# omerkurt-okt/buck-gnn

Hardware: AMD Instinct MI355X
Metric: graphs/sec (fwd+bwd) 6-layer SAGE h=512, ~5k-node meshes, batch 16, 1/2/4/8 GPU (higher is better)
Workload: dtype f32

## Files before the change

### buck-gnn_amd/bgnn/_lib.py

```python
from __future__ import annotations

import ctypes
import os
import threading

_HERE = os.path.dirname(os.path.abspath(__file__))
LIB_PATH = os.environ.get("BGNN_LIBRARY") or os.path.join(_HERE, "_lib", "libbgnn.so")
ABI_VERSION = 16

_lock = threading.Lock()
_lib = None

c_p = ctypes.c_void_p
c_i32 = ctypes.c_int32
c_i64 = ctypes.c_int64
c_f32 = ctypes.c_float
c_u64 = ctypes.c_uint64
c_sz = ctypes.c_size_t


class CsrStruct(ctypes.Structure):

    _fields_ = [
        ("rowptr", c_p),
        ("col", c_p),
        ("heavy_row", c_p),
        ("heavy_chunk0", c_p),
        ("chunk_heavy", c_p),
        ("n_rows", c_i64),
        ("nnz", c_i64),
        ("n_heavy", c_i32),
# ... 100 lines not shown
                                     c_p]),
    "bgnn_gemm_ws_bytes_ex": (c_sz, [c_i64, c_i64, c_i64, c_i32, c_i32, c_i32]),
    "bgnn_gemm_gather_add": (c_i32, [c_i32, c_i32, c_i64, c_i64, c_i64, c_p, c_i64, c_p, c_i64, c_p, c_i64, c_p, c_i32,
                                     c_p, c_p, c_i64, c_p, c_p, c_i64, c_i32, c_p, c_sz, c_p]),
    "bgnn_absmax_f32": (c_i32, [c_p, c_i64, c_i64, c_i64, c_p, c_i32, c_p]),
    "bgnn_gemm_f32_ex": (c_i32, [c_i32, c_i32, c_i64, c_i64, c_i64, c_f32, c_p, c_i64, c_p, c_i64, c_f32, c_p,
                                 c_i64, c_p, c_i32, c_p, c_sz, c_p]),
    "bgnn_topk_rank": (c_i32, [c_p, c_p, c_p, c_i64, c_p, c_p]),
    "bgnn_topk_select": (c_i32, [c_p, c_p, c_p, c_p, c_i64, c_p, c_p, c_p, c_p]),
    "bgnn_gather_scale": (c_i32, [c_p, c_i64, c_i32, c_p, c_p, c_i64, c_p, c_i64, c_p]),
    "bgnn_gather_scale_bwd": (c_i32, [c_p, c_i64, c_p, c_i64, c_i32, c_p, c_p, c_i64, c_p, c_i64, c_p, c_p]),
    "bgnn_filter_edges_ws_bytes": (c_sz, [c_i64]),
    "bgnn_filter_edges": (c_i32, [c_p, c_i64, c_p, c_i64, c_p, c_p, c_p, c_p, c_sz, c_p]),
    "bgnn_mlp2_supported": (c_i32, [c_i32, c_i32, c_i32]),
    "bgnn_mlp2_fwd": (c_i32, [c_p, c_i64, c_i32, c_i32, c_i32, c_p, c_p, c_p, c_p, c_p, c_p, c_p]),
    "bgnn_mlp2_bwd_ws_bytes": (c_sz, [c_i64]),
    "bgnn_mlp2_bwd": (c_i32, [c_p, c_i64, c_i32, c_i32, c_i32, c_p, c_p, c_p, c_p, c_p, c_p, c_p, c_p, c_p, c_p,
                              c_sz, c_p]),
    "bgnn_gemm_f32_dropadd": (c_i32, [c_i32, c_i32, c_i64, c_i64, c_i64, c_p, c_i64, c_p, c_i64, c_p, c_i64, c_p,
                                      c_p, c_p, c_i64, c_f32, c_u64, c_p, c_sz, c_p]),
    "bgnn_gemm_f32_dropadd_cols": (c_i32, [c_i64, c_i64, c_i64, c_p, c_i64, c_p, c_i64, c_p, c_i64, c_p, c_p, c_p,
                                           c_i64, c_i64, c_f32, c_u64, c_p, c_sz, c_p]),
    "bgnn_add_dropout": (c_i32, [c_p, c_p, c_i64, c_f32, c_u64, c_p, c_p]),
    "bgnn_gemm_f32": (c_i32, [c_i32, c_i32, c_i64, c_i64, c_i64, c_f32, c_p, c_i64, c_p, c_i64, c_f32, c_p, c_i64,
                              c_p, c_sz, c_p]),
}


class BgnnError(RuntimeError):
    def __init__(self, fn: str, code: int, msg: str):
        super().__init__(f"{fn} failed with code {code}: {msg}")
        self.code = code


def load():
    global _lib
    if _lib is not None:
        return _lib
    with _lock:
        if _lib is not None:
            return _lib
        if not os.path.exists(LIB_PATH):
            raise ImportError(
                f"bgnn: native library not found at {LIB_PATH}; build it with "
                "`python -c 'import __graft_entry__ as g; g.build()'` or `make -C buck-gnn_amd`")
        lib = ctypes.CDLL(LIB_PATH)
# ... 32 lines not shown
```

### buck-gnn_amd/bgnn/fused.py

```python
from __future__ import annotations

import torch

from . import _lib
from .graph import Graph, _stream, require_cuda

GEMM_BACKEND = "hip"

PLANE_TILE = 128
Z_PLANES = False
DZ_PLANES = False
DGRAD_WT = True
FOLD_WEIGHTS_TORCH = False
DGRAD_DROPADD = True

BF16_PREP = True
ABSMAX_ITEMS = True
PERSISTENT_WPACK = True
MAX_MERGED = True
WSPLIT = True

TIMERS = None
TIMER_EVENT = None


class _timed:
    __slots__ = ("name", "ev")

    def __init__(self, name):
        self.name = name
        self.ev = None

    def __enter__(self):
        if TIMERS is not None:
            mk = TIMER_EVENT or (lambda: torch.cuda.Event(enable_timing=True))
            self.ev = (mk(), mk())
# ... 507 lines not shown
              float(cfg.p), cfg.seed, N, H, x_next.data_ptr(), next_amax.data_ptr(), None, None, s)
    return x_next, (scale, shift, mean, invstd)


def _glue_bwd_stats(g, o, scale, shift, mean, invstd, cfg: LayerConfig, g_rows=None):
    if not cfg.bn:
        return None, None, None, None
    N, H = o.shape
    dev = o.device
    s = _stream()
    rs = _lib.query("bgnn_rows_slots", N)
    part2 = torch.empty(rs, 2, H, dtype=torch.float32, device=dev)
    _lib.call("bgnn_sage_bwd_stats", g.data_ptr(), _ptr(g_rows), o.data_ptr(), scale.data_ptr(), shift.data_ptr(),
              mean.data_ptr(), invstd.data_ptr(), float(cfg.p), cfg.seed, N, H, part2.data_ptr(), s)
    sums = torch.empty(2, H, dtype=torch.float32, device=dev)
    _lib.call("bgnn_reduce_partials", part2.data_ptr(), rs, H, sums[0].data_ptr(), sums[1].data_ptr(), 0, s)
    dbeta, dgamma = sums[0], sums[1]
    if cfg.training:
        return dgamma, dbeta, sums[0], sums[1]
    z = torch.zeros(H, dtype=torch.float32, device=dev)
    return dgamma, dbeta, z, z


class SageLayerFn(torch.autograd.Function):

    @staticmethod
    def forward(ctx, x_prev, x_amax, w_l, b_l, w_r, gamma, beta, running_mean, running_var, graph: Graph,
                cfg: LayerConfig, amax=None, w_in=None, b_in=None, wprep=None, pool=None):
        dev = x_prev.device
        x_prev = x_prev.contiguous()
        H = w_l.size(0)
        N = x_prev.size(0)
        if isinstance(wprep, WPrep):
            wcat, wcat_t_pre, img_f, img_d = wprep.wcat, wprep.wcat_t, wprep, wprep
        elif wprep is not None:
            (wcat, wcat_t_pre), img_f, img_d = wprep, None, None
        else:
            wcat, wcat_t_pre, img_f, img_d = torch.cat([w_l, w_r], 0).contiguous(), None, None, None
        img_f = img_f if (img_f is not None and img_f.img_f is not None) else None
        img_d = img_d if (img_d is not None and img_d.img_d is not None) else None
        if amax is None:
            amax = torch.zeros(3, dtype=torch.float32, device=dev)
        w_amax, next_amax, dz_amax = amax[0:1], amax[1:2], amax[2:3]
        folded = w_in is not None
        if folded:
            if cfg.skip:
                raise ValueError("sage_layer: a folded input transform needs a layer without skip")
            if FOLD_WEIGHTS_TORCH:
                wf = torch.mm(wcat, w_in)
                bf = torch.mv(wcat, b_in)
            else:
                fs = cfg.famax
                fa = (fs[0:1], fs[1:2], fs[2:3]) if fs is not None else (None, None, None)
                if fs is not None:
                    absmax(wcat, fa[0], accumulate=True)
                    absmax(w_in, fa[1], accumulate=True)
                    absmax(b_in.view(1, -1), fa[2], accumulate=True)
                wf = gemm(wcat, w_in.contiguous(), trans_a=False, trans_b=False, a_amax=fa[0], b_amax=fa[1])
                bf = gemm(wcat, b_in.contiguous().view(H, 1), trans_a=False, trans_b=False, a_amax=fa[0],
                          b_amax=fa[2]).view(-1)
            absmax(wf, w_amax, accumulate=True)
            wmat = wf
        else:
            if wprep is None:
                absmax(wcat, w_amax, accumulate=True)
            wmat, bf = wcat, None
        if x_amax is None:
            x_amax = absmax(x_prev)
        planes = Z_PLANES and H % PLANE_TILE == 0 and not folded
        rng = cfg.rng
        x_full = rng.x_full if (rng is not None and rng.x_full is not None and not folded and not planes) else None
        if x_full is not None and x_full.data_ptr() != x_prev.data_ptr():
            raise RuntimeError("sage_layer: RangeRows.x_full must start at x_prev")
        xa, a_amax_g = (x_full, rng.x_amax) if x_full is not None else (x_prev, x_amax)
        M = xa.size(0)
        with _timed("gemm_fwd_fold" if folded else "gemm_fwd"):
            if planes:
                z = torch.empty(2, N, H, dtype=torch.float32, device=dev)
                gemm(x_prev, wmat, trans_a=False, trans_b=True, out=Planes(z), a_amax=x_amax, b_amax=w_amax)
                zl, zr, ldz = z[0], z[1], H
            elif (img_f is not None and not folded
                  and _lib.query("bgnn_gemm_w_tile", M, 2 * H, H) == img_f.bn_f):
                z = torch.empty(M, 2 * H, dtype=torch.float32, device=dev)
                _lib.call("bgnn_gemm_f32_w", M, 2 * H, H, xa.data_ptr(), xa.stride(0), img_f.img_f.data_ptr(),
# ... 4 lines not shown
                z = gemm(xa, wmat, trans_a=False, trans_b=True, bias=bf, a_amax=a_amax_g, b_amax=w_amax)
                zl, zr, ldz = z, z[:, H:], 2 * H
        hagg = z[N:] if x_full is not None else None
        o = torch.empty(N, H, dtype=torch.float32, device=dev)
        nrm = torch.empty(N, dtype=torch.float32, device=dev)
        slots = _lib.query("bgnn_sage_fwd_slots", graph.fwd.ref())
        bn_part = torch.empty(slots, 2, H, dtype=torch.float32, device=dev)
        part = (torch.empty(graph.fwd.plan.n_chunks * H, dtype=torch.float32, device=dev)
                if graph.fwd.plan.n_chunks else None)
        s = _stream()
        with _timed("sage_fwd"):
            _lib.call("bgnn_sage_fwd", graph.fwd.ref(), zl.data_ptr(), ldz, zr.data_ptr(), ldz, b_l.data_ptr(), H,
                      cfg.reduce, o.data_ptr(), nrm.data_ptr(), bn_part.data_ptr(), _ptr(part), _ptr(hagg),
                      2 * H if hagg is not None else 0, s)
        del z, zl, zr, hagg
        x_next, (scale, shift, mean, invstd) = _glue_fwd(o, bn_part, slots, x_prev, gamma, beta, running_mean,
                                                         running_var, cfg, next_amax, graph)
        ctx.graph = graph
        ctx.cfg = cfg
        ctx.folded = folded
        ctx.wcat_t = wcat_t_pre
        ctx.img_d = img_d if not folded else None
        ctx.set_materialize_grads(False)
        ctx.fold = (w_in, b_in, wf) if folded else None
        ctx.save_for_backward(x_prev, o, nrm, wcat, gamma if gamma is not None else torch.empty(0, device=dev),
                              scale if scale is not None else torch.empty(0, device=dev),
                              shift if shift is not None else torch.empty(0, device=dev),
                              mean if mean is not None else torch.empty(0, device=dev),
                              invstd if invstd is not None else torch.empty(0, device=dev),
                              x_amax, w_amax, dz_amax)
        ctx.mark_non_differentiable(next_amax)
        ctx.pool = pool
        if pool is not None:
            from .ops import spmm_fwd
            pooled, _ = spmm_fwd(pool.fwd, x_next, 1, pool.num_rows)
            return x_next, next_amax, pooled
        return x_next, next_amax

    @staticmethod
    def backward(ctx, g, _g_amax, g_pool=None):
        cfg: LayerConfig = ctx.cfg
        g_rows = None
        if g_pool is not None:
            seg = ctx.pool
            gp = g_pool.contiguous() / seg.fwd.degree().clamp_min(1).to(g_pool.dtype).unsqueeze(1)
            if g is None and not cfg.skip:
                g, g_rows = gp, seg.index
# ... 28 lines not shown
              if rb else None)
        _lib.call("bgnn_sage_bwd_rows", g.data_ptr(), _ptr(g_rows), o.data_ptr(), nrm.data_ptr(),
                  _ptr(scale) if bn else None, _ptr(shift) if bn else None,
                  _ptr(gamma) if (bn and gamma.numel()) else None,
                  _ptr(mean) if bn else None, _ptr(invstd) if bn else None, _ptr(sum_g2), _ptr(sum_g2xhat),
                  float(cfg.p), cfg.seed, int(cfg.skip and not dropadd), N, H, dh.data_ptr(), lddz, _ptr(gskip),
                  part_db.data_ptr(), dz_amax.data_ptr(), graph.fwd.rowptr.data_ptr() if ctx.folded else None,
                  (2 if cfg.reduce == 1 else 1) if ctx.folded else 0, _ptr(bw.ranges) if rb else None,
                  graph.fwd.rowptr.data_ptr() if (rb and cfg.reduce == 1) else None, _ptr(rp), s)
        if rb:
            _lib.call("bgnn_range_sums_finish", rp.data_ptr(), N, H, bw.ref(), 1, dzl.data_ptr(), lddz, None,
                      dz_amax.data_ptr(), s)
        db2 = torch.empty(2 if ctx.folded else 1, H, dtype=torch.float32, device=dev)
        _lib.call("bgnn_reduce_partials", part_db.data_ptr(), rs, H, db2[-1].data_ptr(),
                  db2[0].data_ptr() if ctx.folded else None, 0, s)
        db, db_zl = db2[-1], (db2[0] if ctx.folded else None)
        part = torch.empty(bw.plan.n_chunks * H, dtype=torch.float32, device=dev) if bw.plan.n_chunks else None
        with _timed("spmm_bwd"):
            _lib.call("bgnn_spmm_bwd", bw.ref(), graph.perm_t.data_ptr(), graph.fwd.rowptr.data_ptr(),
                      dh.data_ptr(), lddz, H, cfg.reduce, dzl.data_ptr(), lddz, _ptr(part),
                      dz_amax.data_ptr(), int(rb), s)
        has_affine = bn and gamma.numel() > 0
        if ctx.folded:
            w_in, b_in, wf = ctx.fold
            wf_t = wf.t().contiguous() if DGRAD_WT else wf
            with _timed("gemm_dgrad_fold"):
                dx = gemm(dz, wf_t, trans_a=False, trans_b=DGRAD_WT, a_amax=dz_amax, b_amax=w_amax)
            fs = cfg.famax
            fa = (fs[0:1], fs[1:2], fs[2:3], fs[3:4], fs[4:5]) if fs is not None else (None,) * 5
            with _timed("gemm_wgrad_fold"):
                dwf = gemm(dz, x_prev, trans_a=True, trans_b=False, a_amax=dz_amax, b_amax=x_amax,
                           c_amax=fa[3])
            dbf = db2.view(-1)
            if fs is not None:
                absmax(db2, fa[4], accumulate=True)
            if FOLD_WEIGHTS_TORCH:
                dw = torch.addmm(torch.outer(dbf, b_in), dwf, w_in.t())
                dw_in = torch.mm(wcat.t(), dwf)
                db_in = torch.mv(wcat.t(), dbf)
            else:
                dw = gemm(dwf, w_in.contiguous(), trans_a=False, trans_b=True, a_amax=fa[3],
                          b_amax=fa[1])
                dw.add_(torch.outer(dbf, b_in))
                dw_in = gemm(wcat, dwf, trans_a=True, trans_b=False, a_amax=fa[0], b_amax=fa[3])
                db_in = gemm(wcat, dbf.view(-1, 1), trans_a=True, trans_b=False, a_amax=fa[0],
                             b_amax=fa[4]).view(-1)
            return (dx, None, dw[:H], db, dw[H:], dgamma if has_affine else None, dbeta if has_affine else None,
                    None, None, None, None, None, dw_in, db_in, None, None)
        wcat_t = (ctx.wcat_t if ctx.wcat_t is not None else wcat.t().contiguous()) if DGRAD_WT else wcat
        img_d = ctx.img_d if (not planes and DGRAD_WT) else None
        if (img_d is not None and (dropadd or gskip is None)
                and _lib.query("bgnn_gemm_w_tile", N, H, 2 * H) == img_d.bn_d):
            dx = torch.empty(N, H, dtype=torch.float32, device=dev)
            with _timed("gemm_dgrad"):
                _lib.call("bgnn_gemm_f32_w", N, H, 2 * H, dz.data_ptr(), lddz, img_d.img_d.data_ptr(), img_d.bn_d,
                          dx.data_ptr(), H, None, 0, dz_amax.data_ptr(), w_amax.data_ptr(), None,
                          g.data_ptr() if dropadd else None, H, float(cfg.p) if dropadd else 0.0,
                          cfg.seed if dropadd else 0, s)
        elif dropadd:
# ... 503 lines not shown
```

### buck-gnn_amd/csrc/gemm.hip

```cpp
#include "common.h"
#include "gemm_common.h"

namespace bgnn {

extern int g_x6_bdma;

template <int KCONTIG, int BK>
struct Pad {
    static constexpr int value = KCONTIG ? (BK == 16 ? 2 : 1) : 4;
};

template <int KCONTIG, int R, int BK, int NT, bool FULL = false>
__device__ __forceinline__ void load_slice(const float* __restrict__ P, int64_t ld, int64_t Rlim, int64_t r0,
                                           int64_t k0, int64_t kend, bool vec_ok, float (&reg)[R * BK / 4 / NT][4]) {
    constexpr int NL = R * BK / 4 / NT;
    const int t = threadIdx.x;
#pragma unroll
    for (int i = 0; i < NL; ++i) {
        const int idx = t + NT * i;
        if constexpr (FULL) {
            const int r = KCONTIG ? idx / (BK / 4) : (idx % (R / 4)) * 4;
            const int k = KCONTIG ? (idx % (BK / 4)) * 4 : idx / (R / 4);
            const float* src = KCONTIG ? P + (r0 + r) * ld + (k0 + k) : P + (k0 + k) * ld + (r0 + r);
            const float4 v = *reinterpret_cast<const float4*>(src);
// ... 331 lines not shown
        p.prec = 1;
        p.cfg = g_gemm_cfg >= 0 ? g_gemm_cfg % kNumX6Cfgs : pick_x6_cfg(M, N, K, p.prec, ta == 0 && tb == 1);
        if (p.cfg == 5 && !(ta == 0 && tb == 1)) p.cfg = 1;
#ifdef BGNN_H3P_ABLATION
        if (wb && g_x6_bdma == 4 && g_gemm_cfg < 0 && N % 128 == 0 && K % 32 == 0) p.cfg = 0;
#endif
        if (!planes_ok(kX6Cfgs[p.cfg].bm, kX6Cfgs[p.cfg].bn, 32)) {
            p.cfg = 0;
            for (int c = 1; c <= 2; ++c)
                if (planes_ok(kX6Cfgs[c].bm, kX6Cfgs[c].bn, 32)) { p.cfg = c; break; }
        }
        p.bm = kX6Cfgs[p.cfg].bm; p.bn = kX6Cfgs[p.cfg].bn; p.bk = 32;
        p.split = choose_split(M, N, K, GemmCfg{p.bm, p.bn, p.bk, kX6Cfgs[p.cfg].waves,
                                                 kX6Cfgs[p.cfg].blocks_per_cu});
        return p;
    } else {
        p.cfg = pick_cfg(M, N, K, ta, tb);
        if (!planes_ok(kCfgs[p.cfg].bm, kCfgs[p.cfg].bn, kCfgs[p.cfg].bk)) p.cfg = 0;
        const GemmCfg& c = kCfgs[p.cfg];
        p.bm = c.bm; p.bn = c.bn; p.bk = c.bk;
        p.split = choose_split(M, N, K, c);
    }
    return p;
}

constexpr size_t kAmaxHead = 256;

static size_t ws_need(const Plan& p, int64_t M, int64_t N) {
    const size_t head = (p.x6 && p.prec == 1) ? kAmaxHead : 0;
    return head + (p.split > 1 ? (size_t)p.split * (size_t)M * (size_t)N * sizeof(float) : 0);
}

static int launch_splitk_reduce(float* slabs, int split, int64_t M, int64_t N, float alpha, float beta, float* C,
                                int64_t ldc, const float* bias, int relu, int64_t c_blk, int64_t c_pstride,
                                hipStream_t s) {
    int64_t blocks = (M * N + 255) / 256;
    if (blocks > 4096) blocks = 4096;
    int stride = 1;
    const int64_t eb = (M * N + 255) / 256;
    if (split >= 16 && eb < 512) {
        int64_t groups = (512 + eb - 1) / eb;
        if (groups > split / 4) groups = split / 4;
        if (groups >= 2) {
            stride = (int)((split + groups - 1) / groups);
            groups = (split + stride - 1) / stride;
            hipLaunchKernelGGL(k_splitk_stage1, dim3((unsigned)eb, (unsigned)groups), dim3(256), 0, s, slabs, split,
// ... 193 lines not shown
        GemmArgs gb{A, B, C, nullptr, M, N, K, lda, ldb, ldc, 1.f, 0.f, K, 1, bias, relu,
                    0, 0, 0, 0, nullptr, nullptr, nullptr};
        gb.st = st;
        if (b16_ok(gb, ta, tb)) {
            launch_b16(s, gb);
            BGNN_CHECK_LAUNCH();
            return BGNN_OK;
        }
    }
    const int64_t Ma = M;
    GemmArgs g{A, B, C, slabs, Ma, N, K, lda, ldb, ldc, alpha, beta, 0, split, bias, relu,
               a_blk, a_pstride, c_blk, c_pstride, a_amax, b_amax, nullptr};
    g.st = st;
    if (bs.src) {
        g.bsrc = bs.src;
        g.ld_bsrc = bs.ld;
        g.dseed = bs.seed;
        g.dthr = dropout_threshold(bs.p);
        g.dkeep = g.dthr ? 1.f / (1.f - bs.p) : 1.f;
        g.bsrc_c0 = bs.c0;
    }
    const bool c_amax_fused = c_amax != nullptr && pl.x6 && split == 1;
    if (c_amax_fused) g.c_amax = c_amax;
    int64_t kc = (K + split - 1) / split;
    kc = (kc + pl.bk - 1) / pl.bk * pl.bk;
    g.kchunk = kc > 0 ? kc : pl.bk;
    const int64_t tiles_a = ((Ma + pl.bm - 1) / pl.bm) * ((N + pl.bn - 1) / pl.bn);
    dim3 grid((unsigned)tiles_a, split);
    if (pl.x6) launch_x6(pl.prec, ta, tb, pl.cfg, bs.src ? 8 : 0, grid, s, g);
    else if (ta == 0 && tb == 0) launch_cfg<0, 0>(pl.cfg, grid, s, g);
    else if (ta == 0 && tb == 1) launch_cfg<0, 1>(pl.cfg, grid, s, g);
    else if (ta == 1 && tb == 0) launch_cfg<1, 0>(pl.cfg, grid, s, g);
    else launch_cfg<1, 1>(pl.cfg, grid, s, g);
    BGNN_CHECK_LAUNCH();
    if (split > 1) {
        const int rc = launch_splitk_reduce(slabs, split, M, N, alpha, beta, C, ldc, bias, relu, c_blk, c_pstride, s);
        if (rc != BGNN_OK) return rc;
    }
    if (c_amax != nullptr && !c_amax_fused) {
        launch_absmax(C, M, N, ldc, c_blk, c_pstride, c_amax, s);
        BGNN_CHECK_LAUNCH();
    }
    return BGNN_OK;
}

extern "C" int bgnn_gemm_f32_planes(int32_t ta, int32_t tb, int64_t M, int64_t N, int64_t K, float alpha,
                                    const float* A, int64_t lda, int64_t a_blk, int64_t a_pstride, const float* B,
                                    int64_t ldb, float beta, float* C, int64_t ldc, int64_t c_blk,
                                    int64_t c_pstride, const float* bias, int32_t relu, void* ws, size_t ws_bytes,
// ... 140 lines not shown
```

### buck-gnn_amd/csrc/gemm_common.h

```cpp
#pragma once
#include "common.h"

namespace bgnn {

typedef float floatx16 __attribute__((ext_vector_type(16)));
typedef float floatx4 __attribute__((ext_vector_type(4)));

struct GemmArgs {
    const float* A;
    const float* B;
    float* C;
    float* ws;
    int64_t M, N, K, lda, ldb, ldc;
    float alpha, beta;
    int64_t kchunk;
    int split;
    const float* bias;
    int relu;
    int64_t a_blk, a_pstride, c_blk, c_pstride;
    const float* a_amax;
    const float* b_amax;
    float* c_amax;
    const float* ga0; const int64_t* gi0; int64_t ldg0;
    const float* ga1; const int64_t* gi1; int64_t ldg1;
// ... 17 lines not shown
__device__ __forceinline__ void beta_mask4(const GemmArgs& g, int64_t row, int64_t col, const float4& t,
                                           float (&pv)[4]) {
    const int64_t i = row * g.ld_bsrc + col - g.bsrc_c0;
    const uint32_t m = g.dthr ? keep_bits4(g.dseed, (uint64_t)(i >> 2), g.dthr) : 0xFu;
    const float kf = g.dthr ? g.dkeep : 1.f;
    pv[0] = (m & 1u) ? t.x * kf : 0.f;
    pv[1] = (m & 2u) ? t.y * kf : 0.f;
    pv[2] = (m & 4u) ? t.z * kf : 0.f;
    pv[3] = (m & 8u) ? t.w * kf : 0.f;
}

__device__ __forceinline__ const float* plane_base(const float* P, int64_t x0, int64_t blk, int64_t pstride) {
    if (blk <= 0) return P;
    const int64_t plane = x0 / blk;
    return P + plane * (pstride - blk);
}

struct X6Cfg {
    int bm, bn, waves, blocks_per_cu;
};
extern const X6Cfg kX6Cfgs[];
extern const int kNumX6Cfgs;
void launch_x6(int prec, int ta, int tb, int cfg, int abl, dim3 grid, hipStream_t s, const GemmArgs& g);
bool b16_ok(const GemmArgs& g, int ta, int tb);
void launch_b16(hipStream_t s, const GemmArgs& g);
bool b16_dropadd_ok(const GemmArgs& g);
void launch_absmax(const float* P, int64_t rows, int64_t cols, int64_t ld, int64_t blk, int64_t pstride,
                   float* out, hipStream_t s);

}
```

### include/bgnn.h

```cpp
#ifndef BGNN_H
#define BGNN_H

#include <stddef.h>
#include <stdint.h>

#ifdef __cplusplus
extern "C" {
#endif

#define BGNN_ABI_VERSION 16

#define BGNN_OK 0
#define BGNN_E_ARG 1001
#define BGNN_E_WS 1002
#define BGNN_E_UNSUPPORTED 1003

#define BGNN_REDUCE_SUM 0
#define BGNN_REDUCE_MEAN 1
#define BGNN_REDUCE_MAX 2

int bgnn_abi_version(void);
const char* bgnn_last_error_string(void);

#define BGNN_TUNE_SEG_KERNEL 1
#define BGNN_TUNE_SEG_BLOCKS 2
#define BGNN_TUNE_SEG_U 3
#define BGNN_TUNE_SEG_NT 4
#define BGNN_TUNE_GEMM_MODE 5
#define BGNN_TUNE_ROWS_NT 6
#define BGNN_TUNE_GROUP_BLOCKS 7
#define BGNN_TUNE_ROWS_REV 13
#define BGNN_TUNE_GEMM_BDMA 16
int bgnn_heavy_timing(int32_t enable);
// ... 176 lines not shown
                               int64_t ldb, float* C, int64_t ldc, const float* a_amax, const float* b_amax,
                               const float* src, int64_t ld_src, int64_t src_col0, float p, uint64_t seed, void* ws,
                               size_t ws_bytes, void* stream);
int32_t bgnn_gemm_w_tile(int64_t M, int64_t N, int64_t K);
size_t bgnn_gemm_wsplit_bytes(int64_t N, int64_t K);
int bgnn_gemm_wsplit(const float* W, int32_t n_items, int64_t item_stride, int64_t N, int64_t K, int64_t ldw,
                     const float* amax, int64_t amax_stride, void* img, int64_t img_stride, int32_t bn,
                     void* stream);
int bgnn_gemm_f32_w(int64_t M, int64_t N, int64_t K, const float* A, int64_t lda, const void* wimg, int32_t bn,
                    float* C, int64_t ldc, const float* bias, int32_t relu, const float* a_amax,
                    const float* b_amax, float* c_amax, const float* src, int64_t ld_src, float p, uint64_t seed,
                    void* stream);
size_t bgnn_gemm_ws_bytes_ex(int64_t M, int64_t N, int64_t K, int32_t trans_a, int32_t trans_b,
                             int32_t precision);
int bgnn_gemm_gather_add(int32_t trans_a, int32_t trans_b, int64_t M, int64_t N, int64_t K,
                         const float* A, int64_t lda, const float* B, int64_t ldb, float* C, int64_t ldc,
                         const float* bias, int32_t relu, const float* add0, const int64_t* idx0, int64_t ld0,
                         const float* add1, const int64_t* idx1, int64_t ld1, int32_t precision,
                         void* ws, size_t ws_bytes, void* stream);
int bgnn_absmax_f32(const float* x, int64_t rows, int64_t cols, int64_t ld, float* out,
                    int32_t accumulate, void* stream);
int bgnn_absmax_items_f32(const float* x, int32_t n_items, int64_t item_stride, int64_t rows, int64_t cols,
                          int64_t ld, float* out, int64_t out_stride, void* stream);
int bgnn_gemm_f32_planes(int32_t trans_a, int32_t trans_b, int64_t M, int64_t N, int64_t K,
                         float alpha, const float* A, int64_t lda, int64_t a_blk, int64_t a_pstride,
                         const float* B, int64_t ldb, float beta, float* C, int64_t ldc,
                         int64_t c_blk, int64_t c_pstride, const float* bias, int32_t relu,
                         void* ws, size_t ws_bytes, void* stream);

int bgnn_store_gather_graph(const int64_t* table, int32_t B, int64_t Nb, int64_t Eb,
                            int64_t max_nodes, int64_t max_edges,
                            const int32_t* edge_index, int64_t ld_ei,
                            const int32_t* rowptr, const int32_t* col,
                            const int32_t* rowptr_t, const int32_t* col_t, const int32_t* perm_t,
                            int64_t* edge_index_out, int32_t* rowptr_out, int32_t* col_out,
                            int32_t* rowptr_t_out, int32_t* col_t_out, int32_t* perm_t_out,
                            int64_t* batch_out, void* stream);
int bgnn_store_gather_groups(const int64_t* gtable, int32_t B, int32_t group_rows, int64_t Nb, int64_t Gb,
                             int64_t max_edges, int64_t max_groups,
                             const int32_t* gsrc, const uint8_t* gmask, const int32_t* gcnt,
                             const int32_t* gsrc_t, const uint8_t* gmask_t, const int32_t* gcnt_t,
                             int32_t* gsrc_out, uint8_t* gmask_out, int32_t* gcnt_out,
                             int32_t* gsrc_t_out, uint8_t* gmask_t_out, int32_t* gcnt_t_out,
                             int32_t* grow_out, void* stream);
int bgnn_store_gather_rows(const int64_t* table, int32_t B, int32_t per_edge, int64_t max_rows,
                           const void* src, int64_t row_bytes, void* dst, void* stream);
// ... 52 lines not shown
```

Baseline: 2080.

## Fuse folded-input weight products into grouped native HIP kernels

Adds a native fold-weights path that computes the folded weight and bias products, their absmax, and the transposed copy in a single grouped multi-problem kernel launch, with a separate launch for operand maxima. The backward pass does the same for dW, dW_in and db_in, using split-K slabs and a reduce kernel. This replaces several separate gemm, absmax and transpose launches per folded layer. The cost removed is launch count and redundant passes over small weight matrices. It adds a large amount of new kernel code and extra workspace allocations.

```diff
diff --git a/buck-gnn_amd/bgnn/_lib.py b/buck-gnn_amd/bgnn/_lib.py
--- a/buck-gnn_amd/bgnn/_lib.py
+++ b/buck-gnn_amd/bgnn/_lib.py
@@ -6,7 +6,7 @@
 
 _HERE = os.path.dirname(os.path.abspath(__file__))
 LIB_PATH = os.environ.get("BGNN_LIBRARY") or os.path.join(_HERE, "_lib", "libbgnn.so")
-ABI_VERSION = 16
+ABI_VERSION = 17
 
 _lock = threading.Lock()
 _lib = None
@@ -153,6 +153,12 @@
     "bgnn_gemm_f32_dropadd_cols": (c_i32, [c_i64, c_i64, c_i64, c_p, c_i64, c_p, c_i64, c_p, c_i64, c_p, c_p, c_p,
                                            c_i64, c_i64, c_f32, c_u64, c_p, c_sz, c_p]),
     "bgnn_add_dropout": (c_i32, [c_p, c_p, c_i64, c_f32, c_u64, c_p, c_p]),
+    "bgnn_fold_weights_supported": (c_i32, [c_i64, c_i64]),
+    "bgnn_fold_weights_ws_bytes": (c_sz, [c_i64, c_i64]),
+    "bgnn_fold_weights_fwd": (c_i32, [c_i64, c_i64, c_p, c_i64, c_p, c_i64, c_p, c_p, c_p, c_i64, c_p, c_p, c_i64,
+                                      c_p, c_p]),
+    "bgnn_fold_weights_bwd": (c_i32, [c_i64, c_i64, c_p, c_i64, c_p, c_p, c_i64, c_p, c_i64, c_p, c_p, c_p, c_i64,
+                                      c_p, c_i64, c_p, c_p, c_sz, c_p]),
     "bgnn_gemm_f32": (c_i32, [c_i32, c_i32, c_i64, c_i64, c_i64, c_f32, c_p, c_i64, c_p, c_i64, c_f32, c_p, c_i64,
                               c_p, c_sz, c_p]),
 }
diff --git a/buck-gnn_amd/bgnn/fused.py b/buck-gnn_amd/bgnn/fused.py
--- a/buck-gnn_amd/bgnn/fused.py
+++ b/buck-gnn_amd/bgnn/fused.py
@@ -12,6 +12,7 @@
 DZ_PLANES = False
 DGRAD_WT = True
 FOLD_WEIGHTS_TORCH = False
+FOLD_NATIVE = True
 DGRAD_DROPADD = True
 
 BF16_PREP = True
@@ -565,6 +566,12 @@
     return dgamma, dbeta, z, z
 
 
+def _fold_native_ok(famax, wcat, w_in, b_in) -> bool:
+    return bool(FOLD_NATIVE and GEMM_BACKEND == "hip" and famax is not None and famax.is_contiguous()
+                and famax.numel() >= 5 and wcat.stride(1) == 1 and w_in.stride(1) == 1 and b_in.is_contiguous()
+                and _lib.query("bgnn_fold_weights_supported", wcat.size(1), w_in.size(1)))
+
+
 class SageLayerFn(torch.autograd.Function):
 
     @staticmethod
@@ -589,9 +596,19 @@
         if folded:
             if cfg.skip:
                 raise ValueError("sage_layer: a folded input transform needs a layer without skip")
+            wf_t = None
+            fold_native = not FOLD_WEIGHTS_TORCH and _fold_native_ok(cfg.famax, wcat, w_in, b_in)
             if FOLD_WEIGHTS_TORCH:
                 wf = torch.mm(wcat, w_in)
                 bf = torch.mv(wcat, b_in)
+            elif fold_native:
+                K_in = w_in.size(1)
+                wf = torch.empty(2 * H, K_in, dtype=torch.float32, device=dev)
+                bf = torch.empty(2 * H, dtype=torch.float32, device=dev)
+                wf_t = torch.empty(K_in, 2 * H, dtype=torch.float32, device=dev) if DGRAD_WT else None
+                _lib.call("bgnn_fold_weights_fwd", H, K_in, wcat.data_ptr(), wcat.stride(0), w_in.data_ptr(),
+                          w_in.stride(0), b_in.data_ptr(), cfg.famax.data_ptr(), wf.data_ptr(), K_in, bf.data_ptr(),
+                          _ptr(wf_t), 2 * H, w_amax.data_ptr(), _stream())
             else:
                 fs = cfg.famax
                 fa = (fs[0:1], fs[1:2], fs[2:3]) if fs is not None else (None, None, None)
@@ -602,7 +619,8 @@
                 wf = gemm(wcat, w_in.contiguous(), trans_a=False, trans_b=False, a_amax=fa[0], b_amax=fa[1])
                 bf = gemm(wcat, b_in.contiguous().view(H, 1), trans_a=False, trans_b=False, a_amax=fa[0],
                           b_amax=fa[2]).view(-1)
-            absmax(wf, w_amax, accumulate=True)
+            if not fold_native:
+                absmax(wf, w_amax, accumulate=True)
             wmat = wf
         else:
             if wprep is None:
@@ -653,7 +671,7 @@
         ctx.wcat_t = wcat_t_pre
         ctx.img_d = img_d if not folded else None
         ctx.set_materialize_grads(False)
-        ctx.fold = (w_in, b_in, wf) if folded else None
+        ctx.fold = (w_in, b_in, wf, wf_t) if folded else None
         ctx.save_for_backward(x_prev, o, nrm, wcat, gamma if gamma is not None else torch.empty(0, device=dev),
                               scale if scale is not None else torch.empty(0, device=dev),
                               shift if shift is not None else torch.empty(0, device=dev),
@@ -728,8 +746,8 @@
                       dz_amax.data_ptr(), int(rb), s)
         has_affine = bn and gamma.numel() > 0
         if ctx.folded:
-            w_in, b_in, wf = ctx.fold
-            wf_t = wf.t().contiguous() if DGRAD_WT else wf
+            w_in, b_in, wf, wf_t = ctx.fold
+            wf_t = (wf_t if wf_t is not None else wf.t().contiguous()) if DGRAD_WT else wf
             with _timed("gemm_dgrad_fold"):
                 dx = gemm(dz, wf_t, trans_a=False, trans_b=DGRAD_WT, a_amax=dz_amax, b_amax=w_amax)
             fs = cfg.famax
@@ -738,9 +756,21 @@
                 dwf = gemm(dz, x_prev, trans_a=True, trans_b=False, a_amax=dz_amax, b_amax=x_amax,
                            c_amax=fa[3])
             dbf = db2.view(-1)
-            if fs is not None:
+            fold_native = not FOLD_WEIGHTS_TORCH and _fold_native_ok(fs, wcat, w_in, b_in) and dwf.stride(1) == 1
+            if fs is not None and not fold_native:
                 absmax(db2, fa[4], accumulate=True)
-            if FOLD_WEIGHTS_TORCH:
+            if fold_native:
+                K_in = w_in.size(1)
+                dw = torch.empty(2 * H, H, dtype=torch.float32, device=dev)
+                dw_in = torch.empty(H, K_in, dtype=torch.float32, device=dev)
+                db_in = torch.empty(H, dtype=torch.float32, device=dev)
+                ws_bytes = _lib.query("bgnn_fold_weights_ws_bytes", H, K_in)
+                ws = torch.empty(ws_bytes, dtype=torch.uint8, device=dev) if ws_bytes else None
+                _lib.call("bgnn_fold_weights_bwd", H, K_in, dwf.data_ptr(), dwf.stride(0), dbf.data_ptr(),
+                          wcat.data_ptr(), wcat.stride(0), w_in.data_ptr(), w_in.stride(0), b_in.data_ptr(),
+                          fs.data_ptr(), dw.data_ptr(), H, dw_in.data_ptr(), K_in, db_in.data_ptr(), _ptr(ws),
+                          ws_bytes, s)
+            elif FOLD_WEIGHTS_TORCH:
                 dw = torch.addmm(torch.outer(dbf, b_in), dwf, w_in.t())
                 dw_in = torch.mm(wcat.t(), dwf)
                 db_in = torch.mv(wcat.t(), dbf)
diff --git a/buck-gnn_amd/csrc/fold.hip b/buck-gnn_amd/csrc/fold.hip
--- /dev/null
+++ b/buck-gnn_amd/csrc/fold.hip
@@ -0,0 +1,417 @@
+#include "gemm_x6_kernel.h"
+
+namespace bgnn {
+
+constexpr int FNT = 256;
+constexpr int FSL = 4;
+constexpr int f_u4(int rows) { return 2 * rows * 4; }
+
+struct FoldProb {
+    const float* A;
+    const float* B;
+    float* C;
+    float* slabs;
+    int64_t M, N, K, lda, ldb, ldc, kchunk;
+    int split, ta, tb;
+    const float* a_amax;
+    const float* b_amax;
+    int tiles_n, tiles, wg0;
+};
+
+struct FoldArgs {
+    FoldProb p[3];
+    int np;
+    float alpha;
+    float* c_amax;
+    float* ct;
+    int64_t ldct;
+    const float* ou;
+    const float* ov;
+    const float* vmax_src;
+    int64_t vmax_n;
+};
+
+__device__ __forceinline__ bool dev_aligned16(const void* p) { return ((uintptr_t)p & 15) == 0; }
+
+template <int KC, int R>
+struct FoldStage {
+    static constexpr int NQ = R * FSL / FNT;
+    static_assert(KC || (NQ >= 1 && R * FSL % FNT == 0), "k-major operand: whole quads per thread");
+    float v[KC ? FSL : NQ][KC ? x6_nu(R, FNT) : 4][8];
+
+    __device__ __forceinline__ void load(const float* __restrict__ P, int64_t ld, int64_t Rlim, int64_t r0, int64_t k0,
+                                         int64_t s0, int64_t nk, int64_t ke, bool vec_ok, int t) {
+        if constexpr (KC) {
+#pragma unroll
+            for (int u = 0; u < FSL; ++u)
+                if (s0 + u < nk) x6_load<1, R, FNT, false>(P, ld, Rlim, r0, k0 + (s0 + u) * X6_BK, ke, vec_ok, v[u], t);
+        } else {
+#pragma unroll
+            for (int j = 0; j < NQ; ++j) {
+                const int g = t + FNT * j, u = g / R, q = g % R;
+                if (s0 + u < nk) kq_load<R, false>(P, ld, Rlim, r0, k0 + (s0 + u) * X6_BK, ke, vec_ok, v[j], q);
+            }
+        }
+    }
+    __device__ __forceinline__ void store(uint4* __restrict__ S, int stride, int64_t s0, int64_t nk, float sc, int t) {
+        if constexpr (KC) {
+#pragma unroll
+            for (int u = 0; u < FSL; ++u)
+                if (s0 + u < nk) x6_store<1, R, FNT, 1>(S + u * stride, v[u], t, sc);
+        } else {
+#pragma unroll
+            for (int j = 0; j < NQ; ++j) {
+                const int g = t + FNT * j, u = g / R, q = g % R;
+                if (s0 + u < nk) kq_store<R, 1>(S + u * stride, v[j], q, sc);
+            }
+        }
+    }
+};
+
+template <int WM, int WN, int AK, int BK>
+__device__ __forceinline__ void fold_mainloop(const FoldProb& P, int64_t m0, int64_t n0, int64_t kb, int64_t ke,
+                                              float sa, float sb, uint4* __restrict__ smem, bool active,
+                                              floatx16 (&acc)[1][1]) {
+    constexpr int BM = 32 * WM, BN = 32 * WN, A_U4 = f_u4(BM), B_U4 = f_u4(BN);
+    const int t = threadIdx.x, lane = t & 63, wave = t >> 6, wm = wave / WN, wn = wave % WN;
+    const int li = lane & 31, lh = lane >> 5;
+    const bool a_vec = dev_aligned16(P.A) && P.lda % 4 == 0;
+    const bool b_vec = dev_aligned16(P.B) && P.ldb % 4 == 0;
+    const int64_t nk = ke > kb ? (ke - kb + X6_BK - 1) / X6_BK : 0;
+    FoldStage<AK, BM> ra;
+    FoldStage<BK, BN> rb;
+    ra.load(P.A, P.lda, P.M, m0, kb, 0, nk, ke, a_vec, t);
+    rb.load(P.B, P.ldb, P.N, n0, kb, 0, nk, ke, b_vec, t);
+    for (int64_t s0 = 0; s0 < nk; s0 += FSL) {
+        ra.store(smem, A_U4 + B_U4, s0, nk, sa, t);
+        rb.store(smem + A_U4, A_U4 + B_U4, s0, nk, sb, t);
+        __syncthreads();
+        if (s0 + FSL < nk) {
+            ra.load(P.A, P.lda, P.M, m0, kb, s0 + FSL, nk, ke, a_vec, t);
+            rb.load(P.B, P.ldb, P.N, n0, kb, s0 + FSL, nk, ke, b_vec, t);
+        }
+        if (active) {
+#pragma unroll
+            for (int u = 0; u < FSL; ++u) {
+                if (s0 + u < nk) {
+                    const uint4* As = smem + u * (A_U4 + B_U4);
+                    const uint4* Bs = As + A_U4;
+#pragma unroll
+                    for (int kk = 0; kk < X6_BK / 16; ++kk) {
+                        uint4 a[1][2], b[1][2];
+#pragma unroll
+                        for (int p = 0; p < 2; ++p) {
+                            a[0][p] = As[p * BM * 4 + x6_pos(wm * 32 + li, 2 * kk + lh)];
+                            b[0][p] = Bs[p * BN * 4 + x6_pos(wn * 32 + li, 2 * kk + lh)];
+                        }
+                        x6_mma<1, 1, 1, 2>(acc, a, b);
+                    }
+                }
+            }
+        }
+        __syncthreads();
+    }
+}
+
+template <int WM, int WN>
+__global__ __launch_bounds__(FNT) void k_fold_products(FoldArgs fa) {
+    static_assert(WM * WN * 64 == FNT, "four waves");
+    constexpr int BM = 32 * WM, BN = 32 * WN;
+    __shared__ uint4 smem[FSL * (f_u4(BM) + f_u4(BN))];
+    __shared__ uint32_t red[4];
+    int pi = 0;
+#pragma unroll
+    for (int q = 1; q < 3; ++q)
+        if (q < fa.np && (int)blockIdx.x >= fa.p[q].wg0) pi = q;
+    const FoldProb& P = fa.p[pi];
+    const int local = (int)blockIdx.x - P.wg0;
+    const int lt = local % P.tiles, ks = local / P.tiles;
+    const int64_t m0 = (int64_t)(lt / P.tiles_n) * BM, n0 = (int64_t)(lt % P.tiles_n) * BN;
+    const int64_t kb = (int64_t)ks * P.kchunk;
+    const int64_t ke = min(P.K, kb + P.kchunk);
+    const int t = threadIdx.x, lane = t & 63, wave = t >> 6, wm = wave / WN, wn = wave % WN;
+
+    float amax_a = *P.a_amax, amax_b = *P.b_amax;
+    const bool own_vmax = fa.vmax_src != nullptr && pi == fa.np - 1;
+    if (own_vmax) {
+        uint32_t m = __float_as_uint(amax_b);
+        for (int64_t i = t; i < fa.vmax_n; i += FNT) m = max(m, __float_as_uint(fa.vmax_src[i]) & 0x7fffffffu);
+        for (int o = 32; o > 0; o >>= 1) m = max(m, (uint32_t)__shfl_xor((int)m, o, kWave));
+        if (lane == 0) red[wave] = m;
+        __syncthreads();
+        m = max(max(red[0], red[1]), max(red[2], red[3]));
+        amax_b = __uint_as_float(m);
+        if (local == 0 && t == 0 && m) atomicMax(reinterpret_cast<uint32_t*>(const_cast<float*>(P.b_amax)), m);
+    }
+    float sa, sb, ia, ib;
+    h3_scale(amax_a, sa, ia);
+    h3_scale(amax_b, sb, ib);
+
+    floatx16 acc[1][1];
+#pragma unroll
+    for (int r = 0; r < 16; ++r) acc[0][0][r] = 0.f;
+    const int64_t r0 = m0 + wm * 32, c0 = n0 + wn * 32;
+    const bool active = r0 < P.M && c0 < P.N;
+    if constexpr (WM == 1) {
+        fold_mainloop<WM, WN, 1, 0>(P, m0, n0, kb, ke, sa, sb, smem, active, acc);
+    } else {
+        if (P.ta == 0 && P.tb == 0) fold_mainloop<WM, WN, 1, 0>(P, m0, n0, kb, ke, sa, sb, smem, active, acc);
+        else if (P.ta == 0) fold_mainloop<WM, WN, 1, 1>(P, m0, n0, kb, ke, sa, sb, smem, active, acc);
+        else fold_mainloop<WM, WN, 0, 0>(P, m0, n0, kb, ke, sa, sb, smem, active, acc);
+    }
+    if (!active) return;
+
+    const bool split = P.split > 1;
+    float* dst = split ? P.slabs + (int64_t)ks * P.M * P.N : P.C;
+    const int64_t ldd = split ? P.N : P.ldc;
+    const bool vec = dev_aligned16(dst) && ldd % 4 == 0;
+    const bool fast = !split && vec && (r0 & ~(int64_t)63) + 64 <= P.M && (c0 & ~(int64_t)63) + 64 <= P.N;
+    const float iab = ia * ib;
+    const bool one_mul = iab != 0.f && iab < 3.0e38f;
+    const int li = lane & 31, lh = lane >> 5;
+    const int64_t col = c0 + li;
+    const bool first = pi == 0;
+    const bool outer = first && fa.ou != nullptr && !split;
+    const float ovc = (outer && col < P.N) ? fa.ov[col] : 0.f;
+    uint32_t cmax = 0;
+    float vals[16];
+#pragma unroll
+    for (int r = 0; r < 16; ++r) {
+        const int64_t row = r0 + (r & 3) + 8 * (r >> 2) + 4 * lh;
+        const float e = acc[0][0][r];
+        float v;
+        if (split) {
+            v = (e * ia) * ib;
+        } else {
+            v = (fast && one_mul) ? e * iab : (e * ia) * ib;
+            v *= fa.alpha;
+            if (outer && row < P.M) v = __fadd_rn(v, __fmul_rn(fa.ou[row], ovc));
+        }
+        vals[r] = v;
+        if (row < P.M && col < P.N) {
+            dst[row * ldd + col] = v;
+            cmax = max(cmax, __float_as_uint(v) & 0x7fffffffu);
+        }
+    }
+    if (first && fa.ct != nullptr && !split && col < P.N) {
+        const bool tvec = dev_aligned16(fa.ct) && fa.ldct % 4 == 0;
+#pragma unroll
+        for (int q = 0; q < 4; ++q) {
+            const int64_t row = r0 + 8 * q + 4 * lh;
+            float* p = fa.ct + col * fa.ldct + row;
+            if (tvec && row + 3 < P.M) {
+                *reinterpret_cast<float4*>(p) = make_float4(vals[4 * q], vals[4 * q + 1], vals[4 * q + 2], vals[4 * q + 3]);
+            } else {
+#pragma unroll
+                for (int k = 0; k < 4; ++k)
+                    if (row + k < P.M) p[k] = vals[4 * q + k];
+            }
+        }
+    }
+    if (first && fa.c_amax != nullptr && !split) {
+        for (int o = 32; o > 0; o >>= 1) cmax = max(cmax, (uint32_t)__shfl_xor((int)cmax, o, kWave));
+        if (lane == 0 && cmax) atomicMax(reinterpret_cast<uint32_t*>(fa.c_amax), cmax);
+    }
+}
+
+__global__ __launch_bounds__(256) void k_fold_reduce(FoldArgs fa, int64_t e1, int64_t e2) {
+    const int64_t i0 = (int64_t)blockIdx.x * 256 + threadIdx.x;
+    if (i0 >= e2) return;
+    const int pi = i0 < e1 ? 1 : 2;
+    const FoldProb& P = fa.p[pi];
+    const int64_t i = i0 < e1 ? i0 : i0 - e1;
+    const int64_t total = P.M * P.N;
+    float s = 0.f;
+    for (int k = 0; k < P.split; ++k) s += P.slabs[(int64_t)k * total + i];
+    P.C[(i / P.N) * P.ldc + i % P.N] = fa.alpha * s;
+}
+
+struct FoldMaxArgs {
+    const float* P[3];
+    int64_t rows[3], cols[3], ld[3];
+    int b0[4];
+    uint32_t* out;
+};
+
+__global__ __launch_bounds__(256) void k_fold_maxima(FoldMaxArgs a) {
+    int pi = 0;
+    if ((int)blockIdx.x >= a.b0[1]) pi = 1;
+    if ((int)blockIdx.x >= a.b0[2]) pi = 2;
+    const float* __restrict__ P = a.P[pi];
+    const int64_t rows = a.rows[pi], cols = a.cols[pi], ld = a.ld[pi];
+    const int64_t nb = a.b0[pi + 1] - a.b0[pi], b = (int)blockIdx.x - a.b0[pi];
+    uint32_t m = 0;
+    if (cols % 4 == 0 && ld % 4 == 0 && dev_aligned16(P)) {
+        const int64_t c4 = cols / 4, n4 = rows * c4;
+        for (int64_t i = b * 256 + threadIdx.x; i < n4; i += nb * 256) {
+            const float4 v = *reinterpret_cast<const float4*>(P + (i / c4) * ld + (i % c4) * 4);
+            m = max(m, max(max(__float_as_uint(v.x) & 0x7fffffffu, __float_as_uint(v.y) & 0x7fffffffu),
+                           max(__float_as_uint(v.z) & 0x7fffffffu, __float_as_uint(v.w) & 0x7fffffffu)));
+        }
+    } else {
+        const int64_t n = rows * cols;
+        for (int64_t i = b * 256 + threadIdx.x; i < n; i += nb * 256)
+            m = max(m, __float_as_uint(P[(i / cols) * ld + i % cols]) & 0x7fffffffu);
+    }
+    for (int o = 32; o > 0; o >>= 1) m = max(m, (uint32_t)__shfl_xor((int)m, o, kWave));
+    __shared__ uint32_t red[4];
+    if ((threadIdx.x & 63) == 0) red[threadIdx.x >> 6] = m;
+    __syncthreads();
+    if (threadIdx.x == 0) {
+        m = max(max(red[0], red[1]), max(red[2], red[3]));
+        if (m) atomicMax(a.out + pi, m);
+    }
+}
+
+static bool fold_prob(FoldProb& P, int bm, int bn, bool split_ok, int ta, int tb, int64_t M, int64_t N, int64_t K,
+                      const float* A, int64_t lda, const float* B, int64_t ldb, float* C, int64_t ldc,
+                      const float* a_amax, const float* b_amax, int& wg) {
+    int split = 1;
+    int64_t kchunk = 0;
+    if (!small_h3_plan(M, N, K, ta, tb, &split, &kchunk) || split >= 16 || (split > 1 && !split_ok)) return false;
+    P = FoldProb{A, B, C, nullptr, M, N, K, lda, ldb, ldc, kchunk, split, ta, tb, a_amax, b_amax, 0, 0, 0};
+    P.tiles_n = (int)((N + bn - 1) / bn);
+    P.tiles = (int)((M + bm - 1) / bm) * P.tiles_n;
+    P.wg0 = wg;
+    wg += P.tiles * split;
+    return true;
+}
+
+static bool fold_plan_fwd(FoldArgs& fa, int& wg, int64_t H, int64_t K_in, const float* wcat, int64_t ld_wcat,
+                          const float* w_in, int64_t ld_win, const float* b_in, float* fold_amax, float* wf,
+                          int64_t ld_wf, float* bf) {
+    wg = 0;
+    fa.np = 2;
+    return fold_prob(fa.p[0], 32, 128, false, 0, 0, 2 * H, K_in, H, wcat, ld_wcat, w_in, ld_win, wf, ld_wf, fold_amax,
+                     fold_amax + 1, wg) &&
+           fold_prob(fa.p[1], 32, 128, false, 0, 0, 2 * H, 1, H, wcat, ld_wcat, b_in, 1, bf, 1, fold_amax,
+                     fold_amax + 2, wg);
+}
+
+static bool fold_plan_bwd(FoldArgs& fa, int& wg, int64_t H, int64_t K_in, const float* dwf, int64_t ld_dwf,
+                          const float* dbf, const float* wcat, int64_t ld_wcat, const float* w_in, int64_t ld_win,
+                          float* fold_amax, float* dwcat, int64_t ld_dwcat, float* dw_in, int64_t ld_dwin,
+                          float* db_in) {
+    wg = 0;
+    fa.np = 3;
+    return fold_prob(fa.p[0], 64, 64, false, 0, 1, 2 * H, H, K_in, dwf, ld_dwf, w_in, ld_win, dwcat, ld_dwcat,
+                     fold_amax + 3, fold_amax + 1, wg) &&
+           fold_prob(fa.p[1], 64, 64, true, 1, 0, H, K_in, 2 * H, wcat, ld_wcat, dwf, ld_dwf, dw_in, ld_dwin, fold_amax,
+                     fold_amax + 3, wg) &&
+           fold_prob(fa.p[2], 64, 64, true, 1, 0, H, 1, 2 * H, wcat, ld_wcat, dbf, 1, db_in, 1, fold_amax,
+                     fold_amax + 4, wg);
+}
+
+static bool fold_supported(int64_t H, int64_t K_in) {
+    if (H <= 0 || K_in <= 0 || H > 4096 || K_in > 4096 || gemm_mode() != 2) return false;
+    FoldArgs fa{};
+    int wg = 0;
+    float slots[5];
+    return fold_plan_fwd(fa, wg, H, K_in, nullptr, H, nullptr, K_in, nullptr, slots, nullptr, K_in, nullptr) &&
+           fold_plan_bwd(fa, wg, H, K_in, nullptr, K_in, nullptr, nullptr, H, nullptr, K_in, slots, nullptr, H,
+                         nullptr, K_in, nullptr);
+}
+
+}
+
+using namespace bgnn;
+
+extern "C" int32_t bgnn_fold_weights_supported(int64_t H, int64_t K_in) { return fold_supported(H, K_in) ? 1 : 0; }
+
+extern "C" size_t bgnn_fold_weights_ws_bytes(int64_t H, int64_t K_in) {
+    if (!fold_supported(H, K_in)) return 0;
+    FoldArgs fa{};
+    int wg = 0;
+    float slots[5];
+    fold_plan_bwd(fa, wg, H, K_in, nullptr, K_in, nullptr, nullptr, H, nullptr, K_in, slots, nullptr, H, nullptr, K_in,
+                  nullptr);
+    size_t n = 0;
+    if (fa.p[1].split > 1) n += (size_t)fa.p[1].split * H * K_in;
+    if (fa.p[2].split > 1) n += (size_t)fa.p[2].split * H;
+    return n * sizeof(float);
+}
+
+extern "C" int bgnn_fold_weights_fwd(int64_t H, int64_t K_in, const float* wcat, int64_t ld_wcat, const float* w_in,
+                                     int64_t ld_win, const float* b_in, float* fold_amax, float* wf, int64_t ld_wf,
+                                     float* bf, float* wf_t, int64_t ld_wft, float* w_amax, void* stream) {
+    BGNN_REQUIRE(wcat && w_in && b_in && fold_amax && wf && bf && w_amax, "fold_weights_fwd: null pointer");
+    BGNN_REQUIRE(H > 0 && K_in > 0, "fold_weights_fwd: H and K_in must be positive (got %lld, %lld)", (long long)H,
+                 (long long)K_in);
+    BGNN_REQUIRE(ld_wcat >= H && ld_win >= K_in && ld_wf >= K_in && (!wf_t || ld_wft >= 2 * H),
+                 "fold_weights_fwd: a leading dimension is shorter than its row");
+    FoldArgs fa{};
+    int wg = 0;
+    BGNN_REQUIRE(fold_supported(H, K_in) &&
+                     fold_plan_fwd(fa, wg, H, K_in, wcat, ld_wcat, w_in, ld_win, b_in, fold_amax, wf, ld_wf, bf),
+                 "fold_weights_fwd: H=%lld, K_in=%lld unsupported (bgnn_fold_weights_supported)", (long long)H,
+                 (long long)K_in);
+    hipStream_t s = as_stream(stream);
+    FoldMaxArgs ma{};
+    ma.P[0] = wcat; ma.rows[0] = 2 * H; ma.cols[0] = H; ma.ld[0] = ld_wcat;
+    ma.P[1] = w_in; ma.rows[1] = H; ma.cols[1] = K_in; ma.ld[1] = ld_win;
+    ma.P[2] = b_in; ma.rows[2] = 1; ma.cols[2] = H; ma.ld[2] = H;
+    ma.b0[0] = 0;
+    for (int q = 0; q < 3; ++q) {
+        int64_t nb = (ma.rows[q] * ma.cols[q] + 8191) / 8192;
+        nb = nb < 1 ? 1 : (nb > 64 ? 64 : nb);
+        ma.b0[q + 1] = ma.b0[q] + (int)nb;
+    }
+    ma.out = reinterpret_cast<uint32_t*>(fold_amax);
+    hipLaunchKernelGGL(k_fold_maxima, dim3((unsigned)ma.b0[3]), dim3(256), 0, s, ma);
+    BGNN_CHECK_LAUNCH();
+    fa.alpha = 1.f;
+    fa.c_amax = w_amax;
+    fa.ct = wf_t;
+    fa.ldct = ld_wft;
+    hipLaunchKernelGGL((k_fold_products<1, 4>), dim3((unsigned)wg), dim3(FNT), 0, s, fa);
+    BGNN_CHECK_LAUNCH();
+    return BGNN_OK;
+}
+
+extern "C" int bgnn_fold_weights_bwd(int64_t H, int64_t K_in, const float* dwf, int64_t ld_dwf, const float* dbf,
+                                     const float* wcat, int64_t ld_wcat, const float* w_in, int64_t ld_win,
+                                     const float* b_in, float* fold_amax, float* dwcat, int64_t ld_dwcat,
+                                     float* dw_in, int64_t ld_dwin, float* db_in, void* ws, size_t ws_bytes,
+                                     void* stream) {
+    BGNN_REQUIRE(dwf && dbf && wcat && w_in && b_in && fold_amax && dwcat && dw_in && db_in,
+                 "fold_weights_bwd: null pointer");
+    BGNN_REQUIRE(H > 0 && K_in > 0, "fold_weights_bwd: H and K_in must be positive (got %lld, %lld)", (long long)H,
+                 (long long)K_in);
+    BGNN_REQUIRE(ld_dwf >= K_in && ld_wcat >= H && ld_win >= K_in && ld_dwcat >= H && ld_dwin >= K_in,
+                 "fold_weights_bwd: a leading dimension is shorter than its row");
+    FoldArgs fa{};
+    int wg = 0;
+    BGNN_REQUIRE(fold_supported(H, K_in) &&
+                     fold_plan_bwd(fa, wg, H, K_in, dwf, ld_dwf, dbf, wcat, ld_wcat, w_in, ld_win, fold_amax, dwcat,
+                                   ld_dwcat, dw_in, ld_dwin, db_in),
+                 "fold_weights_bwd: H=%lld, K_in=%lld unsupported (bgnn_fold_weights_supported)", (long long)H,
+                 (long long)K_in);
+    const size_t need = bgnn_fold_weights_ws_bytes(H, K_in);
+    BGNN_REQUIRE(need == 0 || (ws != nullptr && ws_bytes >= need),
+                 "fold_weights_bwd: workspace of %zu bytes, bgnn_fold_weights_ws_bytes() asks %zu", ws_bytes, need);
+    hipStream_t s = as_stream(stream);
+    float* slabs = static_cast<float*>(ws);
+    int64_t e1 = 0, e2 = 0;
+    if (fa.p[1].split > 1) {
+        fa.p[1].slabs = slabs;
+        slabs += (int64_t)fa.p[1].split * H * K_in;
+        e1 = H * K_in;
+    }
+    e2 = e1;
+    if (fa.p[2].split > 1) {
+        fa.p[2].slabs = slabs;
+        e2 += H;
+    }
+    fa.alpha = 1.f;
+    fa.ou = dbf;
+    fa.ov = b_in;
+    fa.vmax_src = dbf;
+    fa.vmax_n = 2 * H;
+    hipLaunchKernelGGL((k_fold_products<2, 2>), dim3((unsigned)wg), dim3(FNT), 0, s, fa);
+    BGNN_CHECK_LAUNCH();
+    if (e2 > 0) {
+        hipLaunchKernelGGL(k_fold_reduce, dim3((unsigned)((e2 + 255) / 256)), dim3(256), 0, s, fa, e1, e2);
+        BGNN_CHECK_LAUNCH();
+    }
+    return BGNN_OK;
+}
diff --git a/buck-gnn_amd/csrc/gemm.hip b/buck-gnn_amd/csrc/gemm.hip
--- a/buck-gnn_amd/csrc/gemm.hip
+++ b/buck-gnn_amd/csrc/gemm.hip
@@ -377,6 +377,22 @@
         p.split = choose_split(M, N, K, c);
     }
     return p;
+}
+
+static int64_t split_kchunk(int64_t K, int split, int bk) {
+    int64_t kc = (K + split - 1) / split;
+    kc = (kc + bk - 1) / bk * bk;
+    return kc > 0 ? kc : bk;
+}
+
+namespace bgnn {
+bool small_h3_plan(int64_t M, int64_t N, int64_t K, int ta, int tb, int* split, int64_t* kchunk) {
+    const Plan p = make_plan(M, N, K, ta, tb, 0, 0);
+    if (!p.x6 || p.prec != 1 || p.cfg != 0) return false;
+    *split = p.split;
+    *kchunk = split_kchunk(K, p.split, p.bk);
+    return true;
+}
 }
 
 constexpr size_t kAmaxHead = 256;
@@ -616,9 +632,7 @@
     }
     const bool c_amax_fused = c_amax != nullptr && pl.x6 && split == 1;
     if (c_amax_fused) g.c_amax = c_amax;
-    int64_t kc = (K + split - 1) / split;
-    kc = (kc + pl.bk - 1) / pl.bk * pl.bk;
-    g.kchunk = kc > 0 ? kc : pl.bk;
+    g.kchunk = split_kchunk(K, split, pl.bk);
     const int64_t tiles_a = ((Ma + pl.bm - 1) / pl.bm) * ((N + pl.bn - 1) / pl.bn);
     dim3 grid((unsigned)tiles_a, split);
     if (pl.x6) launch_x6(pl.prec, ta, tb, pl.cfg, bs.src ? 8 : 0, grid, s, g);
diff --git a/buck-gnn_amd/csrc/gemm_common.h b/buck-gnn_amd/csrc/gemm_common.h
--- a/buck-gnn_amd/csrc/gemm_common.h
+++ b/buck-gnn_amd/csrc/gemm_common.h
@@ -63,6 +63,7 @@
 extern const X6Cfg kX6Cfgs[];
 extern const int kNumX6Cfgs;
 void launch_x6(int prec, int ta, int tb, int cfg, int abl, dim3 grid, hipStream_t s, const GemmArgs& g);
+bool small_h3_plan(int64_t M, int64_t N, int64_t K, int ta, int tb, int* split, int64_t* kchunk);
 bool b16_ok(const GemmArgs& g, int ta, int tb);
 void launch_b16(hipStream_t s, const GemmArgs& g);
 bool b16_dropadd_ok(const GemmArgs& g);
diff --git a/include/bgnn.h b/include/bgnn.h
--- a/include/bgnn.h
+++ b/include/bgnn.h
@@ -8,7 +8,7 @@
 extern "C" {
 #endif
 
-#define BGNN_ABI_VERSION 16
+#define BGNN_ABI_VERSION 17
 
 #define BGNN_OK 0
 #define BGNN_E_ARG 1001
@@ -231,6 +231,15 @@
                     int32_t accumulate, void* stream);
 int bgnn_absmax_items_f32(const float* x, int32_t n_items, int64_t item_stride, int64_t rows, int64_t cols,
                           int64_t ld, float* out, int64_t out_stride, void* stream);
+int32_t bgnn_fold_weights_supported(int64_t H, int64_t K_in);
+size_t bgnn_fold_weights_ws_bytes(int64_t H, int64_t K_in);
+int bgnn_fold_weights_fwd(int64_t H, int64_t K_in, const float* wcat, int64_t ld_wcat, const float* w_in,
+                          int64_t ld_win, const float* b_in, float* fold_amax, float* wf, int64_t ld_wf,
+                          float* bf, float* wf_t, int64_t ld_wft, float* w_amax, void* stream);
+int bgnn_fold_weights_bwd(int64_t H, int64_t K_in, const float* dwf, int64_t ld_dwf, const float* dbf,
+                          const float* wcat, int64_t ld_wcat, const float* w_in, int64_t ld_win,
+                          const float* b_in, float* fold_amax, float* dwcat, int64_t ld_dwcat, float* dw_in,
+                          int64_t ld_dwin, float* db_in, void* ws, size_t ws_bytes, void* stream);
 int bgnn_gemm_f32_planes(int32_t trans_a, int32_t trans_b, int64_t M, int64_t N, int64_t K,
                          float alpha, const float* A, int64_t lda, int64_t a_blk, int64_t a_pstride,
                          const float* B, int64_t ldb, float beta, float* C, int64_t ldc,
```

New measurement: 2110, median of 6. 1.01x the previous value.
